# thucz/splatter360

Measured on AMD Instinct MI355X. Metric: Msplats/s fwd+bwd @1M Gaussians, 1024x512 ERP, higher is better.
Workload: dtype f32; 1 GPU; BASELINE configs[2]: 1048576 encoder-like synthetic Gaussians (seed 0, deg-4 SH, from 2 context panoramas 1024x512), 1024x512 ERP = 6 faces 256x256 + stitch, fwdbwd, L2 loss on faces (fused epilogue, scalar reduced in the backward's first launch), lean tile lists; gaussians=1048576, face=256, views_per_gpu=1, parallelism=view-sharded x1, num_rendered=2237238, visible_pairs=1096454, split_lists=auto, split_quadrants=0, wide_rectangles=0, workspace_bytes_forward=1086434304, workspace_bytes_backward=1062934272, max_instances=2862083

## Files before the change

### splatter360_amd/csrc/s360_device.h

```cpp
#pragma once
#include <hip/hip_runtime.h>
#include <stdint.h>

#include "../../include/s360.h"

#define S360_WAVE 64
#define S360_BLOCK 256

#ifndef S360_SUB_W
#define S360_SUB_W 8
#endif

static inline int s360_effective_degree(const S360Params* prm) {
    return (prm->sh_degree > 3 && (prm->flags & S360_FLAG_SH_DEG4_IGNORED)) ? 3 : prm->sh_degree;
}

#ifndef S360_PREC_F4
#define S360_PREC_F4 4
#endif

namespace s360 {

constexpr int PREC_F4 = S360_PREC_F4;
constexpr int SUB_W = S360_SUB_W, SUB_H = 64 / S360_SUB_W;
__device__ __forceinline__ int sub_ox(int w) { return SUB_W == 16 ? 0 : 8 * (w & 1); }
__device__ __forceinline__ int sub_oy(int w) { return SUB_W == 16 ? 4 * w : 8 * (w >> 1); }


struct KParams {
    int P, V, H, W, deg, M;
    int gx, gy, T;
    uint32_t flags, cap;
};

#ifndef S360_SEG_LEN
#define S360_SEG_LEN 512
#endif
#ifndef S360_SEG_HEAD
#define S360_SEG_HEAD 1024
#endif
#ifndef S360_SEG_BWD_BLOCKS
#define S360_SEG_BWD_BLOCKS 256
#endif
#ifndef S360_SEG_MIN_REST
#define S360_SEG_MIN_REST 512
#endif
constexpr uint32_t SEG_LEN = S360_SEG_LEN, SEG_HEAD = S360_SEG_HEAD, SEG_MIN_REST = S360_SEG_MIN_REST, SEG_PER_CHUNK = 4096 / SEG_LEN;
constexpr uint32_t SEG_K0 = SEG_HEAD / SEG_LEN;
static_assert(4096 % SEG_LEN == 0 && SEG_HEAD % SEG_LEN == 0 && SEG_LEN % 64 == 0 && SEG_K0 >= 1, "segments tile the sort's 4 096-key chunks; slot 0 holds the head's state");
__device__ constexpr float SEG_T_FAR = 1.0f / 16.0f;
__host__ __device__ inline size_t seg_slots(size_t cap) { return (size_t)SEG_PER_CHUNK * (cap / 2048 + 1); }
__host__ __device__ inline size_t seg_slots_of(const S360Params* prm) {
    return prm->max_segments ? (size_t)prm->max_segments : seg_slots(prm->max_instances ? prm->max_instances : 1);
}
#define S360_HDR_SPLIT 5
#define S360_HDR_SEGWORK 6
#define S360_HDR_TILES_DONE 24
#define S360_HDR_NLONG 25
#define S360_SEG_CLAIM 0x80000000u
#define S360_HDR_SEGBUFS 32

inline int device_cu_count() {
    static int cached[64] = {};
    int dev = 0;
    if (hipGetDevice(&dev) != hipSuccess || dev < 0 || dev >= 64) return 256;
    if (!cached[dev]) {
        int n = 0;
        if (hipDeviceGetAttribute(&n, hipDeviceAttributeMultiprocessorCount, dev) != hipSuccess || n <= 0) { (void)hipGetLastError(); n = 256; }
        cached[dev] = n;
    }
    return cached[dev];
}

inline int resident_blocks(const void* fn, int block_threads, int slot) {
    static int cached[64][16] = {};
    int dev = 0;
    if (hipGetDevice(&dev) != hipSuccess || dev < 0 || dev >= 64 || slot < 0 || slot >= 16) return 4 * 256;
    if (!cached[dev][slot]) {
        int per_cu = 0;
        if (hipOccupancyMaxActiveBlocksPerMultiprocessor(&per_cu, fn, block_threads, 0) != hipSuccess || per_cu <= 0) { (void)hipGetLastError(); per_cu = 4; }
        cached[dev][slot] = per_cu * device_cu_count();
    }
    return cached[dev][slot];
}

__device__ constexpr float kC0 = 0.28209479177387814f;
__device__ constexpr float kC1 = 0.4886025119029199f;
__device__ constexpr float kC2[5] = {1.0925484305920792f, -1.0925484305920792f, 0.31539156525252005f,
                                     -1.0925484305920792f, 0.5462742152960396f};
__device__ constexpr float kC3[7] = {-0.5900435899266435f, 2.890611442640554f, -0.4570457994644658f,
                                     0.3731763325901154f, -0.4570457994644658f, 1.445305721320277f,
                                     -0.5900435899266435f};
__device__ constexpr float kC4[9] = {2.5033429417967046f, -1.7701307697799304f, 0.9461746957575601f,
                                     -0.6690465435572892f, 0.10578554691520431f, -0.6690465435572892f,
                                     0.47308734787878004f, -1.7701307697799304f, 0.6258357354491761f};

__device__ __forceinline__ void sh_basis(int deg, float x, float y, float z, float* Y) {
    Y[0] = kC0;
    if (deg > 0) {
        Y[1] = -kC1 * y;
        Y[2] = kC1 * z;
        Y[3] = -kC1 * x;
        if (deg > 1) {
            float xx = x * x, yy = y * y, zz = z * z, xy = x * y, yz = y * z, xz = x * z;
            Y[4] = kC2[0] * xy;
            Y[5] = kC2[1] * yz;
            Y[6] = kC2[2] * (2.0f * zz - xx - yy);
            Y[7] = kC2[3] * xz;
            Y[8] = kC2[4] * (xx - yy);
            if (deg > 2) {
                Y[9] = kC3[0] * y * (3.0f * xx - yy);
                Y[10] = kC3[1] * xy * z;
                Y[11] = kC3[2] * y * (4.0f * zz - xx - yy);
                Y[12] = kC3[3] * z * (2.0f * zz - 3.0f * xx - 3.0f * yy);
                Y[13] = kC3[4] * x * (4.0f * zz - xx - yy);
                Y[14] = kC3[5] * z * (xx - yy);
                Y[15] = kC3[6] * x * (xx - 3.0f * yy);
// ... 537 lines not shown
```

### splatter360_amd/csrc/s360_forward.hip

```cpp
#include "s360_device.h"
#include "s360_prof.h"
#include "s360_adapter_math.h"

#include <cstdio>
#include <cstdlib>

namespace s360 {

typedef float f4v __attribute__((ext_vector_type(4)));

template <bool CH_MAJOR, bool JAC>
__global__ __launch_bounds__(S360_BLOCK) void k_sh_eval(KParams kp, const S360View* __restrict__ views,
                                                       const float* __restrict__ means, const float* __restrict__ shs,
                                                       float4* __restrict__ rgbc, float* __restrict__ sh_jac,
                                                       uint32_t* __restrict__ zero_ptr, int zero_words) {
    const int g = blockIdx.x * S360_BLOCK + threadIdx.x;
    if (g < zero_words) zero_ptr[g] = 0u;
    if (g >= kp.P) return;
    const bool fast = kp.M == 25 && kp.deg == 4;
    const float* sh = shs + (size_t)g * kp.M * 3;
    float c[75];
    if (fast) load75(sh, c);
    const S360View& vw = views[0];
    const float sc = vw.scale;
// ... 326 lines not shown
#pragma unroll
        for (int a = 0; a < 3; ++a)
#pragma unroll
            for (int b = a; b < 3; ++b) S[a][b] = S[b][a] = M[a][0] * s2[0] * M[b][0] + M[a][1] * s2[1] * M[b][1] + M[a][2] * s2[2] * M[b][2];
        float* oc = rin.cov6_out + 6 * (size_t)g;
        oc[0] = S[0][0]; oc[1] = S[0][1]; oc[2] = S[0][2]; oc[3] = S[1][1]; oc[4] = S[1][2]; oc[5] = S[2][2];
    }
    if (d == 2 && live && rin.geo7) {
        const float* rw = s_raw + l * RAW_C;
        float* o7 = rin.geo7 + 7 * (size_t)g;
#pragma unroll
        for (int k = 0; k < 7; ++k) o7[k] = rw[k];
    }
    __syncthreads();
    if (JAC) {
        const int gl = tid / 3, ch = tid - 3 * gl;
        if (gl < nb) {
            const float G0 = s_G[(3 * ch) * SHE3_G + gl], G1 = s_G[(3 * ch + 1) * SHE3_G + gl], G2 = s_G[(3 * ch + 2) * SHE3_G + gl];
            const float4 dr = s_dir[gl];
            const float dot = dr.x * G0 + dr.y * G1 + dr.z * G2;
            float* o = sh_jac + 3 * ((size_t)g0 * 3 + tid);
            o[0] = (G0 - dr.x * dot) * dr.w;
            o[1] = (G1 - dr.y * dot) * dr.w;
            o[2] = (G2 - dr.z * dot) * dr.w;
        }
    }
    if (tid < nb) {
        const float a0 = s_rgb[3 * tid], a1 = s_rgb[3 * tid + 1], a2 = s_rgb[3 * tid + 2];
        const uint32_t clampbits = (a0 < 0.f ? 1u : 0u) | (a1 < 0.f ? 2u : 0u) | (a2 < 0.f ? 4u : 0u);
        rgbc[g0 + tid] = make_float4(fmaxf(a0, 0.f), fmaxf(a1, 0.f), fmaxf(a2, 0.f), __uint_as_float(clampbits));
    }
}

template <bool USE_SH, bool CH_MAJOR, bool EAGER = false, bool COOP = false>
__global__ __launch_bounds__(S360_BLOCK) void k_preprocess(
    KParams kp, const S360View* __restrict__ views, const float* __restrict__ means,
    const float* __restrict__ cov6, const float* __restrict__ opac, const float* __restrict__ shs,
    const float* __restrict__ colors, int32_t* __restrict__ radii, uint32_t* __restrict__ tiles_touched,
    float4* __restrict__ recA, float4* __restrict__ recB, float4* __restrict__ recC,
    uint8_t* __restrict__ clamped, float* __restrict__ depths, uint32_t* __restrict__ tile_count, int lds_hist,
    const float4* __restrict__ rgbc, uint8_t* __restrict__ vis_mask, uint2* __restrict__ slot_info) {
    extern __shared__ __attribute__((aligned(16))) float lds_sh[];
    const int tid = threadIdx.x;
    const int g0 = blockIdx.x * S360_BLOCK;
    const int P = kp.P;
    const bool act = g0 + tid < P;
    const int g = act ? g0 + tid : P - 1;
    uint32_t* hist = reinterpret_cast<uint32_t*>(lds_sh);
    const bool lean = (kp.flags & S360_FLAG_LEAN_LISTS) != 0;
    const int nhist = lds_hist == 2 ? kp.T : (image_of_view(kp, kp.V - 1) + 1) * kp.T;
    if (lds_hist)
        for (int i = tid; i < nhist; i += S360_BLOCK) hist[i] = 0u;

    __syncthreads();
    {
    const float mx0 = means[3 * g], my0 = means[3 * g + 1], mz0 = means[3 * g + 2];
    float c60[6];
    load_cov6(cov6, g, (kp.flags & S360_FLAG_COV9) != 0, c60);
    const float op = opac[g];
    constexpr bool ch_major = CH_MAJOR;

    const bool shared_cam = (kp.flags & S360_FLAG_SHARED_CAMPOS) != 0;
    float rgb[3] = {0.f, 0.f, 0.f};
    uint32_t clampbits = 0;
    bool have_rgb = false;
    if (!USE_SH) {
        rgb[0] = colors[3 * g];
        rgb[1] = colors[3 * g + 1];
        rgb[2] = colors[3 * g + 2];
        have_rgb = true;
    }

    uint32_t vis = 0;
    for (int v = 0; v < kp.V; ++v) {
// ... 165 lines not shown
                for (int i = lane; i < n; i += 64) {
                    const int y = i / w;
                    atomicAdd(&tc[(miny + y) * kp.gx + minx + (i - y * w)], 1u);
                }
            }
        }
        if (act && radii) radii[p] = radius;
        if (touched) {
            tiles_touched[p] = touched;
            vis |= 1u << v;
        }
        if (lds_hist == 2) {
            __syncthreads();
            uint32_t* tcg = tile_count + (size_t)image_of_view(kp, v) * kp.T;
            for (int i = tid; i < nhist; i += S360_BLOCK) {
                const uint32_t c = hist[i];
                if (c) {
                    atomicAdd(&tcg[i], c);
                    hist[i] = 0u;
                }
            }
            __syncthreads();
        }
    }
    if (act) vis_mask[g] = (uint8_t)vis;
    }
    if (lds_hist == 1) {
        __syncthreads();
        for (int i = tid; i < nhist; i += S360_BLOCK) {
            const uint32_t c = hist[i];
            if (c) atomicAdd(&tile_count[i], c);
        }
    }
}


template <int NW = S360_BLOCK / 64>
__device__ __forceinline__ uint32_t block_exclusive_scan(uint32_t v, uint32_t* lds, uint32_t& total) {
    const int lane = lane_id(), wave = threadIdx.x >> 6;
    uint32_t inc = v;
#pragma unroll
    for (int o = 1; o < 64; o <<= 1) {
        uint32_t t = (uint32_t)__shfl_up((int)inc, o);
        if (lane >= o) inc += t;
    }
    if (lane == 63) lds[wave] = inc;
    __syncthreads();
    uint32_t base = 0, tot = 0;
#pragma unroll
    for (int w = 0; w < NW; ++w) {
        const uint32_t s = lds[w];
        if (w < wave) base += s;
        tot += s;
    }
    __syncthreads();
    total = tot;
    return base + inc - v;
}

#ifndef S360_SORT_THREADS
#define S360_SORT_THREADS 512
#endif
constexpr int SORT_THREADS = S360_SORT_THREADS;
constexpr uint32_t SORT_SHORT = 2048;
constexpr uint32_t SORT_CHUNK = 8 * SORT_THREADS;
static_assert(SORT_SHORT % SORT_THREADS == 0 && SORT_SHORT <= SORT_CHUNK, "short lists: SORT_SHORT / SORT_THREADS keys per thread");
constexpr uint32_t MAX_PASSES = 4;
__device__ __forceinline__ uint32_t ceil_log2_u32(uint32_t x) { return x <= 1 ? 0u : 32u - (uint32_t)__builtin_clz(x - 1); }
constexpr uint32_t LDSM_CHUNKS = 4;
constexpr int LDSM_E = 32;
__device__ __forceinline__ uint32_t merge_passes_of(uint32_t nch) { return nch <= 1 ? 0u : nch <= LDSM_CHUNKS ? 1u : ceil_log2_u32(nch); }

struct SegBufs {
    const uint32_t* chunk_start;
    uint32_t* seg_flag;
    uint32_t* seg_arrive;
    uint32_t* seg_arrive2;
    uint32_t n_slots;
    float4* part_c;
    float* part_t;
    float* part_e;
    uint32_t* part_l;
    uint32_t* part_n;
    float4* seg_c;
    float* seg_t;
    uint32_t* seg_cnt;
    uint2* seg_info;
    uint32_t* header;
};
static_assert(sizeof(SegBufs) <= (64 - S360_HDR_SEGBUFS) * 4, "SegBufs is parked in the workspace header");

constexpr int TS_BLOCK = 1024;
__global__ __launch_bounds__(TS_BLOCK) void k_tile_scan(const uint32_t* __restrict__ tile_count, uint32_t* __restrict__ tile_start,
                                                         uint32_t* __restrict__ tile_cursor, uint32_t* __restrict__ tile_max_contrib,
                                                         int nt, uint32_t cap, uint32_t* __restrict__ header,
                                                         uint32_t* __restrict__ chunk_start, unsigned long long* __restrict__ header_mirror,
                                                         SegBufs sg_in) {
    __shared__ uint32_t lds[TS_BLOCK / 64];
    __shared__ uint32_t lds_max, lds_nlong;
    if (threadIdx.x == 0) { lds_max = 0; lds_nlong = 0; }
    __syncthreads();
    uint32_t carry = 0, mx = 0, ccarry = 0;
    for (int b = 0; b < nt; b += 2 * TS_BLOCK) {
        const int i0 = b + 2 * (int)threadIdx.x, i1 = i0 + 1;
        uint32_t v0 = 0u, v1 = 0u;
        if (i1 < nt) {
            const uint2 vv = *reinterpret_cast<const uint2*>(tile_count + i0);
            v0 = vv.x; v1 = vv.y;
        } else if (i0 < nt) {
            v0 = tile_count[i0];
        }
        mx = max(mx, max(v0, v1));
        uint32_t tot;
        const uint32_t ex0 = block_exclusive_scan<TS_BLOCK / 64>(v0 + v1, lds, tot), ex1 = ex0 + v0;
        const uint32_t nc0 = min(carry + ex0 + v0, cap) - min(carry + ex0, cap), nc1 = min(carry + ex1 + v1, cap) - min(carry + ex1, cap);
        const uint32_t nch0 = nc0 > SORT_SHORT ? (nc0 + SORT_CHUNK - 1) / SORT_CHUNK : 0u;
        const uint32_t nch1 = nc1 > SORT_SHORT ? (nc1 + SORT_CHUNK - 1) / SORT_CHUNK : 0u;
        if (nch0 || nch1) atomicAdd(&lds_nlong, (nch0 ? 1u : 0u) + (nch1 ? 1u : 0u));
        uint32_t ctot;
        const uint32_t cex0 = block_exclusive_scan<TS_BLOCK / 64>(nch0 + nch1, lds, ctot), cex1 = cex0 + nch0;
        if (i0 < nt) {
            tile_start[i0] = carry + ex0;
            tile_cursor[i0] = 0;
            tile_max_contrib[i0] = 0;
            chunk_start[i0] = ccarry + cex0;
        }
        if (i1 < nt) {
            tile_start[i1] = carry + ex1;
            tile_cursor[i1] = 0;
            tile_max_contrib[i1] = 0;
            chunk_start[i1] = ccarry + cex1;
        }
        carry += tot;
        ccarry += ctot;
    }
    atomicMax(&lds_max, mx);
    __syncthreads();
    if (threadIdx.x == 0) {
        chunk_start[nt] = ccarry;
        tile_start[nt] = carry;
        header[0] = carry;
        header[1] = carry > cap ? 1u : 0u;
        header[2] = lds_max;
        {
            const uint32_t nmax = min(lds_max, cap);
            const uint32_t nch = nmax > SORT_SHORT ? (nmax + SORT_CHUNK - 1) / SORT_CHUNK : 0u;
            header[3] = merge_passes_of(nch);
        }
        header[4] = 0;
        *reinterpret_cast<SegBufs*>(header + S360_HDR_SEGBUFS) = sg_in;
        header[S360_HDR_SPLIT] = 0;
        header[6] = header[7] = 0;
        if (header_mirror) __hip_atomic_store(header_mirror, (unsigned long long)carry | ((unsigned long long)(carry > cap ? 1u : 0u) << 32) |
                                                             ((unsigned long long)ccarry << 33),
                                              __ATOMIC_RELAXED, __HIP_MEMORY_SCOPE_SYSTEM);
        header[S360_HDR_NLONG] = lds_nlong;
        for (int i = 8; i < 25; ++i) header[i] = 0;
    }
}

#ifndef S360_EMIT_PPT
#define S360_EMIT_PPT 4
#endif
constexpr int EMIT_PPT = S360_EMIT_PPT;

template <bool LDS_BIN, bool COOP = false>
__global__ __launch_bounds__(S360_BLOCK) void k_emit(KParams kp, const uint32_t* __restrict__ tiles_touched,
                                                    const uint8_t* __restrict__ vis_mask, const float4* __restrict__ recA, const float4* __restrict__ recC,
                                                    const float* __restrict__ depths, const uint32_t* __restrict__ tile_start,
                                                    uint32_t* __restrict__ tile_cursor, uint64_t* __restrict__ keys,
                                                    uint2* __restrict__ slot_info, uint32_t* __restrict__ slot_pair,
                                                    uint32_t* __restrict__ slot_ticket, uint32_t* __restrict__ header,
                                                    uint32_t* __restrict__ long_pairs) {
    extern __shared__ __attribute__((aligned(16))) uint32_t lds_bin[];
    __shared__ uint32_t s_scan[S360_BLOCK / 64];
    __shared__ uint32_t s_slot0;
    const int v = blockIdx.y;
    const int g0 = blockIdx.x * (S360_BLOCK * EMIT_PPT) + threadIdx.x;
    const size_t tb = (size_t)image_of_view(kp, v) * kp.T;
    uint32_t* cnt = lds_bin;
    uint32_t* base = lds_bin + kp.T;
    const bool lean = (kp.flags & S360_FLAG_LEAN_LISTS) != 0;
    if (LDS_BIN) {
        for (int i = threadIdx.x; i < kp.T; i += S360_BLOCK) cnt[i] = 0u;
        __syncthreads();
    }
    __shared__ uint32_t s_p[S360_BLOCK * EMIT_PPT];
    uint32_t vis = 0;
#pragma unroll
    for (int j = 0; j < EMIT_PPT; ++j) {
// ... 730 lines not shown
                    const bool stop = mine && test_T < 0.0001f;
                    const bool contrib = mine && !stop;
                    if (!T_ONLY) {
                        const float w = contrib ? a_s * T : 0.0f;
                        C01.x += rl(eb.z, eb_) * w;
                        C01.y += rl(eb.w, eb_) * w;
                        C2D.x += rl(ec, eb_) * w;
                        if (WITH_DEPTH) C2D.y += rl(ez, eb_) * w;
                        last = contrib ? rel + (uint32_t)eb_ + 1u : last;
                    }
                    T = contrib ? test_T : T;
                    done = done || stop;
                    if (__ballot(stop) != 0ull) break;
                }
            }
        }
    }
}

template <bool WITH_DEPTH, bool COH>
__device__ __forceinline__ void seg_item(const KParams& kp, const S360View* __restrict__ views, const uint32_t* __restrict__ tile_start,
                                         const uint32_t* __restrict__ list, const float4* __restrict__ recA, float* __restrict__ images,
                                         float* __restrict__ final_T, uint32_t* __restrict__ n_contrib, uint32_t* __restrict__ tile_max_contrib,
                                         uint32_t* __restrict__ strip_last, const float* __restrict__ depths, float* __restrict__ depth_maps,
                                         int depth_mode, const MseEp& ep, float4* __restrict__ surv, uint32_t* __restrict__ surv_count,
                                         const SegBufs& sg, int nt, uint32_t* __restrict__ dbg, const WaveLds& L, int lane, uint2 item, uint32_t wi,
                                         uint32_t nwork);

#ifndef S360_SPLIT_WAVES
#define S360_SPLIT_WAVES 4
#endif
#ifndef S360_P1_GRID
#define S360_P1_GRID 1024
#endif
#ifndef S360_P1_FIRST
#define S360_P1_FIRST 0
#endif
#ifndef S360_P2_GRID
#define S360_P2_GRID 1024
#endif
#ifndef S360_SEGS_SPINS
#define S360_SEGS_SPINS 600
#endif
template <bool WITH_DEPTH, bool SPLIT>
__global__ __launch_bounds__(S360_BLOCK) __attribute__((amdgpu_waves_per_eu(SPLIT ? S360_SPLIT_WAVES : 6, SPLIT ? S360_SPLIT_WAVES : 6))) void k_render(KParams kp, const S360View* __restrict__ views,
                                                      const uint32_t* __restrict__ tile_start, const uint32_t* __restrict__ list,
                                                      const float4* __restrict__ recA, const float4* __restrict__ recB,
                                                      const float4* __restrict__ recC, float* __restrict__ images,
                                                      float* __restrict__ final_T, uint32_t* __restrict__ n_contrib,
                                                      uint32_t* __restrict__ tile_max_contrib, uint32_t* __restrict__ strip_last,
                                                      uint32_t* __restrict__ dbg, const float* __restrict__ depths,
                                                      float* __restrict__ depth_maps, int depth_mode, MseEp ep,
                                                      const uint32_t* __restrict__ tile_order, float4* __restrict__ surv,
                                                      uint32_t* __restrict__ surv_count, uint32_t* __restrict__ hdr_loss,
                                                      const SegBufs* __restrict__ sgp, const uint32_t* __restrict__ chunk_start,
                                                      unsigned long long* __restrict__ cand_mirror, int nt, const uint32_t* __restrict__ list_all,
                                                      const float* __restrict__ depths_all) {
#ifdef S360_DBG_TIMING
    const long long t_begin = wall_clock64();
#endif
    __shared__ __attribute__((aligned(16))) float s_x[S360_BLOCK / 64][68], s_y[S360_BLOCK / 64][68], s_a[S360_BLOCK / 64][68],
        s_b[S360_BLOCK / 64][68], s_c[S360_BLOCK / 64][68], s_o[S360_BLOCK / 64][68];
    __shared__ __attribute__((aligned(16))) float2 s_rg[S360_BLOCK / 64][68], s_bz[S360_BLOCK / 64][68];
    __shared__ __attribute__((aligned(16))) uint32_t s_pos[S360_BLOCK / 64][68];
    if (hdr_loss && blockIdx.x == 0 && threadIdx.x == 0) {
        const uint64_t pp = (uint64_t)(uintptr_t)ep.partials, po = (uint64_t)(uintptr_t)ep.loss_out;
        hdr_loss[0] = (uint32_t)pp; hdr_loss[1] = (uint32_t)(pp >> 32);
        hdr_loss[2] = (uint32_t)po; hdr_loss[3] = (uint32_t)(po >> 32);
        hdr_loss[4] = (uint32_t)(kp.T * 4); hdr_loss[5] = (uint32_t)kp.V;
        hdr_loss[6] = __float_as_uint(0.5f * ep.grad_scale);
        hdr_loss[7] = __float_as_uint(1.0f / (3.0f * (float)kp.H * (float)kp.W));
        for (int i = 0; i <= kp.V; ++i) ep.loss_out[i] = __uint_as_float(0x7FC00000u);
    }
    __shared__ uint32_t s_retired;
    uint32_t tile_slot = blockIdx.x;
    if (SPLIT) {
        const SegBufs& sgr = *sgp;
        const uint32_t n_long = S360_P1_FIRST ? sgr.header[S360_HDR_NLONG] : (uint32_t)nt;
        const uint32_t b = blockIdx.x;
        if (b >= n_long && b < n_long + (uint32_t)S360_P1_GRID) {
            const SegBufs sg = sgr;
            const int pwave = threadIdx.x >> 6, lane = threadIdx.x & 63;
            const WaveLds L{s_x[pwave], s_y[pwave], s_a[pwave], s_b[pwave], s_c[pwave], s_o[pwave], s_rg[pwave], s_bz[pwave], s_pos[pwave]};
            const uint32_t nunits = min((uint32_t)(SEG_PER_CHUNK * chunk_start[nt]), sg.n_slots);
            for (uint32_t u = b - n_long; u < nunits; u += (uint32_t)S360_P1_GRID) {
#ifdef S360_DBG_TIMING
                const long long t_p1 = wall_clock64();
#endif
                const ChunkUnit cu = chunk_unit(tile_start, chunk_start, nt, kp.cap, u / SEG_PER_CHUNK);
                const uint32_t k = cu.k * SEG_PER_CHUNK + (u % SEG_PER_CHUNK);
                if (!cu.valid || k < SEG_K0 || k * SEG_LEN >= cu.n || cu.n < SEG_HEAD + SEG_MIN_REST) continue;
                const int t1 = (int)cu.t, v1 = t1 / kp.T, rem1 = t1 - v1 * kp.T;
                const int ty1 = rem1 / kp.gx, tx1 = rem1 - ty1 * kp.gx;
                const int px1 = tx1 * 16 + sub_ox(pwave) + lane % SUB_W, py1 = ty1 * 16 + sub_oy(pwave) + lane / SUB_W;
                const bool inside1 = px1 < kp.W && py1 < kp.H;
                float T1 = 1.0f;
                f2 c01 = f2{0.f, 0.f}, c2d = f2{0.f, 0.f};
                uint32_t last1 = 0, cnt1 = 0;
                bool done1 = !inside1;
                const uint32_t b0 = cu.s + k * SEG_LEN, b1 = min(b0 + SEG_LEN, cu.s + cu.n);
                composite_segment<WITH_DEPTH, true>(list, recA, depths, cu.s, b0, b1, (float)px1, (float)py1, (float)(tx1 * 16 + sub_ox(pwave)),
                                                    (float)(ty1 * 16 + sub_oy(pwave)), lane, L, 0.f, 0.f, 0.f, depth_mode, T1, c01, c2d, last1, done1,
                                                    nullptr, cnt1);
                st_devf(sg.part_t + ((size_t)u * 4 + pwave) * 64 + lane, (done1 && inside1) ? 0.0f : T1);
                asm volatile("s_waitcnt vmcnt(0)" ::: "memory");
                if (lane == 0) __hip_atomic_fetch_add(&sg.seg_arrive[4 * t1 + pwave], 1u, __ATOMIC_RELAXED, __HIP_MEMORY_SCOPE_AGENT);
#ifdef S360_DBG_TIMING
                if (lane == 0) {
                    const size_t di = 4 * ((size_t)4 * nt + (size_t)4 * sg.n_slots + (size_t)u * 4 + pwave);
                    dbg[di] = (uint32_t)t_begin; dbg[di + 1] = (uint32_t)t_p1; dbg[di + 2] = (uint32_t)(wall_clock64() - t_p1);
                    dbg[di + 3] = ((uint32_t)t1 << 8) | k;
// ... 709 lines not shown
    if (sph && (kp.V & 1)) return S360_E_BADARG;
    const int nt = (sph ? kp.V / 2 : kp.V) * kp.T;
    const size_t np = (size_t)kp.V * kp.P;

    uint32_t* header = (uint32_t*)(ws + L.header);
    uint32_t* tiles_touched = (uint32_t*)(ws + L.tiles_touched);
    uint8_t* vis_mask = (uint8_t*)(ws + L.vis_mask);
    uint2* slot_info = (uint2*)(ws + L.slot_base);
    uint32_t* slot_ticket = (uint32_t*)(ws + L.slot_ticket);
    float4* recA = (float4*)(ws + L.rec_a);
    float4* recB = (float4*)(ws + L.rec_b);
    float4* recC = (float4*)(ws + L.rec_c);
    uint8_t* clamped = (uint8_t*)(ws + L.clamped);
    float* depths = (float*)(ws + L.depths);
    uint32_t* tile_count = (uint32_t*)(ws + L.tile_count);
    uint32_t* tile_start = (uint32_t*)(ws + L.tile_start);
    uint32_t* tile_cursor = (uint32_t*)(ws + L.tile_cursor);
    uint64_t* keys = (uint64_t*)(ws + L.keys);
    uint64_t* keys_alt = (uint64_t*)(ws + L.keys_alt);
    uint32_t* chunk_start = (uint32_t*)(ws + L.chunk_start);
    uint32_t* tile_order = (uint32_t*)(ws + L.tile_order);
    uint32_t* list = (uint32_t*)(ws + L.list);
    float* final_T = (float*)(ws + L.final_T);
    uint32_t* n_contrib = (uint32_t*)(ws + L.n_contrib);
    uint32_t* tile_max_contrib = (uint32_t*)(ws + L.tile_max_contrib);
    uint32_t* strip_last = (uint32_t*)(ws + L.strip_last);

    const bool eager_sh = kp.P > 0 && shs && (kp.flags & S360_FLAG_SHARED_CAMPOS) && (!(kp.flags & S360_FLAG_FORWARD_ONLY) || kp.V >= 2 || rawin);
    const size_t zero_words_sz = (L.tile_start - L.tile_count) / 4;
    const bool fold_clear = eager_sh && zero_words_sz <= (size_t)kp.P;
    uint32_t* zero_ptr = fold_clear ? tile_count : (uint32_t*)nullptr;
    const int zero_words = fold_clear ? (int)zero_words_sz : 0;
    if (!fold_clear && hipMemsetAsync(tile_count, 0, L.tile_start - L.tile_count, st) != hipSuccess) return S360_E_LAUNCH;
    if (kp.P > 0) {
        {
        const int nblk = (kp.P + S360_BLOCK - 1) / S360_BLOCK;
        const int lds_hist = (size_t)nt * 4 <= 48 * 1024 ? 1 : ((size_t)kp.T * 4 <= 48 * 1024 ? 2 : 0);
        const size_t hist_bytes = lds_hist == 2 ? (size_t)kp.T * 4 : (size_t)nt * 4;
        const bool eager = eager_sh;
        float4* rgbc = (float4*)(ws + L.rgbc);
        if (eager) {
            ProfScope ps(PS_SH_EVAL, st);
            float* sh_jac = (float*)(ws + L.sh_jac);
            const bool jac = !(kp.flags & S360_FLAG_FORWARD_ONLY);
            const bool chm = (kp.flags & S360_FLAG_SH_CHANNEL_MAJOR) != 0;
#define S360_SHE(A, B) hipLaunchKernelGGL((k_sh_eval<A, B>), dim3(nblk), dim3(S360_BLOCK), 0, st, kp, views, means3D, shs, rgbc, sh_jac, zero_ptr, zero_words)
            if (rawin) {
                RawIn rin = *rawin;
                rin.geo7 = jac ? (float*)(ws + L.geo7) : nullptr;
                const dim3 rgrid((rin.Gv + SHE3_G - 1) / SHE3_G, (unsigned)(kp.P / rin.Gv));
                const bool rot = rin.sh_rot != nullptr;
#define S360_RAWE(J, R, M) hipLaunchKernelGGL((k_raw_eval<J, R, M>), rgrid, dim3(SHE3_G * 3), 0, st, kp, views, rin, rgbc, sh_jac, zero_ptr, zero_words)
                static const bool raw_mfma = [] { const char* e = getenv("S360_RAW_MFMA"); return e && e[0] == '1'; }();
                if (rot && raw_mfma) { if (jac) S360_RAWE(true, true, true); else S360_RAWE(false, true, true); }
                else if (jac) { if (rot) S360_RAWE(true, true, false); else S360_RAWE(true, false, false); }
                else { if (rot) S360_RAWE(false, true, false); else S360_RAWE(false, false, false); }
#undef S360_RAWE
            } else if (chm && kp.M == 25 && kp.deg == 4) {
                const int nb3 = (kp.P + SHE3_G - 1) / SHE3_G;
                if (jac) hipLaunchKernelGGL(k_sh_eval3_jac, dim3(nb3), dim3(SHE3_G * 3), 0, st, kp, views, means3D, shs, rgbc, sh_jac, zero_ptr, zero_words);
                else hipLaunchKernelGGL(k_sh_eval3, dim3(nb3), dim3(SHE3_G * 3), 0, st, kp, views, means3D, shs, rgbc, zero_ptr, zero_words);
            } else if (chm && jac) S360_SHE(true, true); else if (chm) S360_SHE(true, false); else if (jac) S360_SHE(false, true); else S360_SHE(false, false);
#undef S360_SHE
        }
        ProfScope ps(PS_PREPROCESS, st);
        if (shs) {
            const size_t lds = lds_hist ? hist_bytes : 0;
            if (eager && (kp.flags & S360_FLAG_COOP_WALK))
                hipLaunchKernelGGL((k_preprocess<true, true, true, true>), dim3(nblk), dim3(S360_BLOCK), lds, st, kp, views, means3D, cov6,
                                   opacities, shs, colors_precomp, radii, tiles_touched, recA, recB, recC, clamped, depths,
                                   tile_count, lds_hist, rgbc, vis_mask, slot_info);
            else if (eager)
                hipLaunchKernelGGL((k_preprocess<true, true, true>), dim3(nblk), dim3(S360_BLOCK), lds, st, kp, views, means3D, cov6,
                                   opacities, shs, colors_precomp, radii, tiles_touched, recA, recB, recC, clamped, depths,
                                   tile_count, lds_hist, rgbc, vis_mask, slot_info);
            else if (kp.flags & S360_FLAG_SH_CHANNEL_MAJOR)
                hipLaunchKernelGGL((k_preprocess<true, true>), dim3(nblk), dim3(S360_BLOCK), lds, st, kp, views, means3D, cov6,
                                   opacities, shs, colors_precomp, radii, tiles_touched, recA, recB, recC, clamped, depths,
                                   tile_count, lds_hist, rgbc, vis_mask, slot_info);
            else
                hipLaunchKernelGGL((k_preprocess<true, false>), dim3(nblk), dim3(S360_BLOCK), lds, st, kp, views, means3D, cov6,
                                   opacities, shs, colors_precomp, radii, tiles_touched, recA, recB, recC, clamped, depths,
                                   tile_count, lds_hist, rgbc, vis_mask, slot_info);
        } else {
            hipLaunchKernelGGL((k_preprocess<false, false>), dim3(nblk), dim3(S360_BLOCK), lds_hist ? hist_bytes : 0, st, kp, views,
                               means3D, cov6, opacities, shs, colors_precomp, radii, tiles_touched, recA, recB, recC, clamped,
                               depths, tile_count, lds_hist, rgbc, vis_mask, slot_info);
        }
        }
        S360_CHECK_LAUNCH();
    }
    {
        ProfScope ps(PS_TILE_SCAN, st);
        const bool split0 = kp.P > 0 && (kp.flags & S360_FLAG_SPLIT_LISTS);
        SegBufs sg0{split0 ? chunk_start : (const uint32_t*)nullptr, (uint32_t*)(ws + L.seg_flag), (uint32_t*)(ws + L.seg_arrive),
                    (uint32_t*)(ws + L.seg_arrive2), (uint32_t)seg_slots_of(prm),
                    (float4*)(ws + L.part_c), (float*)(ws + L.part_t), (float*)(ws + L.part_e), (uint32_t*)(ws + L.part_l), (uint32_t*)(ws + L.part_n),
                    (float4*)(ws + L.seg_c), (float*)(ws + L.seg_t), (uint32_t*)(ws + L.seg_cnt), (uint2*)(ws + L.seg_info), header};
        hipLaunchKernelGGL(k_tile_scan, dim3(1), dim3(TS_BLOCK), 0, st, tile_count, tile_start, tile_cursor, tile_max_contrib, nt, kp.cap, header,
                           chunk_start, (unsigned long long*)prm->header_mirror, sg0);
    }
    S360_CHECK_LAUNCH();
    if (kp.P > 0) {
        const dim3 egrid((kp.P + S360_BLOCK * EMIT_PPT - 1) / (S360_BLOCK * EMIT_PPT), kp.V);
        uint32_t* slot_pair = (kp.flags & S360_FLAG_FORWARD_ONLY) ? nullptr : (uint32_t*)(ws + L.slot_pair);
        {
        ProfScope ps(PS_EMIT, st);
        if ((size_t)kp.T * 8 <= 64 * 1024 && (kp.flags & S360_FLAG_COOP_WALK))
            hipLaunchKernelGGL((k_emit<true, true>), egrid, dim3(S360_BLOCK), (size_t)kp.T * 8, st, kp, tiles_touched, vis_mask, recA, recC,
                               depths, tile_start, tile_cursor, keys, slot_info, slot_pair, slot_ticket, header, (uint32_t*)(ws + L.long_pairs));
        else if ((size_t)kp.T * 8 <= 64 * 1024)
            hipLaunchKernelGGL(k_emit<true>, egrid, dim3(S360_BLOCK), (size_t)kp.T * 8, st, kp, tiles_touched, vis_mask, recA, recC,
                               depths, tile_start, tile_cursor, keys, slot_info, slot_pair, slot_ticket, header, (uint32_t*)(ws + L.long_pairs));
        else
            hipLaunchKernelGGL(k_emit<false>, egrid, dim3(S360_BLOCK), 0, st, kp, tiles_touched, vis_mask, recA, recC, depths, tile_start,
                               tile_cursor, keys, slot_info, slot_pair, slot_ticket, header, (uint32_t*)(ws + L.long_pairs));
        }
        S360_CHECK_LAUNCH();
        ProfScope ps(PS_SORT, st);
        {
            const size_t cap_keys = kp.cap < (uint32_t)kp.P ? kp.cap : (size_t)kp.P;
            uint32_t passes = 0;
            while (passes < MAX_PASSES && ((size_t)SORT_CHUNK << passes) < cap_keys) ++passes;
            const uint32_t global_lo = SORT_CHUNK << passes;
            const unsigned cgrid = (unsigned)min((size_t)1024, (size_t)kp.cap / SORT_CHUNK + (size_t)kp.cap / SORT_SHORT + 2);
            const size_t lds512 = (size_t)(SORT_CHUNK + SORT_CHUNK / 8) * 8;
            hipLaunchKernelGGL(k_sort_stage1, dim3(cgrid + nt + 1), dim3(SORT_THREADS), lds512, st, tile_start, chunk_start, nt, keys, keys_alt, list,
                               kp.cap, passes, cgrid, tile_count, tile_order, header,
                               prm->header_mirror ? (unsigned long long*)prm->header_mirror + 2 : (unsigned long long*)nullptr);
            if (passes > 0) {
                const unsigned mgrid = cgrid < (unsigned)S360_MERGE_GRID ? cgrid : (unsigned)S360_MERGE_GRID;
                {
                    static bool attr_done[64] = {};
// ... 108 lines not shown
```

Baseline: 1355 Msplats/s.

## Fold tile-count scan into the last preprocess workgroup to drop a launch

The single-block tile scan kernel is removed from the normal path. Instead, each preprocess workgroup increments a done counter after its histogram flush, and the last one to finish runs the scan body itself, reading its arguments from the kernarg segment. This removes one kernel launch and the dependency gap before the scan. In exchange the scan runs on a 256-thread block instead of 1024 threads, and the optional long-tile count header field and the P1_FIRST path are dropped.

Result: slower. 1338 Msplats/s (-1.3%).

```diff
diff --git a/splatter360_amd/csrc/s360_device.h b/splatter360_amd/csrc/s360_device.h
--- a/splatter360_amd/csrc/s360_device.h
+++ b/splatter360_amd/csrc/s360_device.h
@@ -56,33 +56,8 @@
 #define S360_HDR_SPLIT 5
 #define S360_HDR_SEGWORK 6
 #define S360_HDR_TILES_DONE 24
-#define S360_HDR_NLONG 25
 #define S360_SEG_CLAIM 0x80000000u
 #define S360_HDR_SEGBUFS 32
-
-inline int device_cu_count() {
-    static int cached[64] = {};
-    int dev = 0;
-    if (hipGetDevice(&dev) != hipSuccess || dev < 0 || dev >= 64) return 256;
-    if (!cached[dev]) {
-        int n = 0;
-        if (hipDeviceGetAttribute(&n, hipDeviceAttributeMultiprocessorCount, dev) != hipSuccess || n <= 0) { (void)hipGetLastError(); n = 256; }
-        cached[dev] = n;
-    }
-    return cached[dev];
-}
-
-inline int resident_blocks(const void* fn, int block_threads, int slot) {
-    static int cached[64][16] = {};
-    int dev = 0;
-    if (hipGetDevice(&dev) != hipSuccess || dev < 0 || dev >= 64 || slot < 0 || slot >= 16) return 4 * 256;
-    if (!cached[dev][slot]) {
-        int per_cu = 0;
-        if (hipOccupancyMaxActiveBlocksPerMultiprocessor(&per_cu, fn, block_threads, 0) != hipSuccess || per_cu <= 0) { (void)hipGetLastError(); per_cu = 4; }
-        cached[dev][slot] = per_cu * device_cu_count();
-    }
-    return cached[dev][slot];
-}
 
 __device__ constexpr float kC0 = 0.28209479177387814f;
 __device__ constexpr float kC1 = 0.4886025119029199f;
diff --git a/splatter360_amd/csrc/s360_forward.hip b/splatter360_amd/csrc/s360_forward.hip
--- a/splatter360_amd/csrc/s360_forward.hip
+++ b/splatter360_amd/csrc/s360_forward.hip
@@ -382,6 +382,195 @@
     }
 }
 
+
+template <int NW = S360_BLOCK / 64>
+__device__ __forceinline__ uint32_t block_exclusive_scan(uint32_t v, uint32_t* lds, uint32_t& total) {
+    const int lane = lane_id(), wave = threadIdx.x >> 6;
+    uint32_t inc = v;
+#pragma unroll
+    for (int o = 1; o < 64; o <<= 1) {
+        uint32_t t = (uint32_t)__shfl_up((int)inc, o);
+        if (lane >= o) inc += t;
+    }
+    if (lane == 63) lds[wave] = inc;
+    __syncthreads();
+    uint32_t base = 0, tot = 0;
+#pragma unroll
+    for (int w = 0; w < NW; ++w) {
+        const uint32_t s = lds[w];
+        if (w < wave) base += s;
+        tot += s;
+    }
+    __syncthreads();
+    total = tot;
+    return base + inc - v;
+}
+
+#ifndef S360_SORT_THREADS
+#define S360_SORT_THREADS 512
+#endif
+constexpr int SORT_THREADS = S360_SORT_THREADS;
+constexpr uint32_t SORT_SHORT = 2048;
+constexpr uint32_t SORT_CHUNK = 8 * SORT_THREADS;
+static_assert(SORT_SHORT % SORT_THREADS == 0 && SORT_SHORT <= SORT_CHUNK, "short lists: SORT_SHORT / SORT_THREADS keys per thread");
+constexpr uint32_t MAX_PASSES = 4;
+__device__ __forceinline__ uint32_t ceil_log2_u32(uint32_t x) { return x <= 1 ? 0u : 32u - (uint32_t)__builtin_clz(x - 1); }
+constexpr uint32_t LDSM_CHUNKS = 4;
+constexpr int LDSM_E = 32;
+__device__ __forceinline__ uint32_t merge_passes_of(uint32_t nch) { return nch <= 1 ? 0u : nch <= LDSM_CHUNKS ? 1u : ceil_log2_u32(nch); }
+
+struct SegBufs {
+    const uint32_t* chunk_start;
+    uint32_t* seg_flag;
+    uint32_t* seg_arrive;
+    uint32_t* seg_arrive2;
+    uint32_t n_slots;
+    float4* part_c;
+    float* part_t;
+    float* part_e;
+    uint32_t* part_l;
+    uint32_t* part_n;
+    float4* seg_c;
+    float* seg_t;
+    uint32_t* seg_cnt;
+    uint2* seg_info;
+    uint32_t* header;
+};
+static_assert(sizeof(SegBufs) <= (64 - S360_HDR_SEGBUFS) * 4, "SegBufs is parked in the workspace header");
+
+__device__ __forceinline__ uint32_t sort_chunks_of(uint32_t nc0) {
+    const uint32_t nch0 = nc0 > SORT_SHORT ? (nc0 + SORT_CHUNK - 1) / SORT_CHUNK : 0u;
+    return nch0;
+}
+
+struct ScanArgs {
+    const uint32_t* tile_count;
+    uint32_t* tile_start;
+    uint32_t* tile_cursor;
+    uint32_t* tile_max_contrib;
+    uint32_t* chunk_start;
+    uint32_t* header;
+    unsigned long long* header_mirror;
+    uint32_t* done;
+    int nt;
+    uint32_t cap;
+    SegBufs sg;
+};
+
+__device__ __forceinline__ uint32_t ld_count(const uint32_t* p) { return __hip_atomic_load(p, __ATOMIC_RELAXED, __HIP_MEMORY_SCOPE_AGENT); }
+
+template <int THREADS>
+__device__ __forceinline__ void tile_scan_body(const ScanArgs& sa, uint32_t* lds) {
+    constexpr int PER = 8;
+    uint32_t* lds_max = lds + THREADS / 64;
+    if (threadIdx.x == 0) *lds_max = 0;
+    __syncthreads();
+    const int nt = sa.nt;
+    const uint32_t cap = sa.cap;
+    uint32_t carry = 0, mx = 0, ccarry = 0;
+    for (int b = 0; b < nt; b += PER * THREADS) {
+        const int i0 = b + PER * (int)threadIdx.x;
+        uint32_t v[PER], sum = 0;
+#pragma unroll
+        for (int k = 0; k < PER; ++k) v[k] = i0 + k < nt ? ld_count(sa.tile_count + i0 + k) : 0u;
+#pragma unroll
+        for (int k = 0; k < PER; ++k) {
+            mx = max(mx, v[k]);
+            sum += v[k];
+        }
+        uint32_t tot;
+        const uint32_t ex = carry + block_exclusive_scan<THREADS / 64>(sum, lds, tot);
+        uint32_t nch[PER], csum = 0, off = ex;
+#pragma unroll
+        for (int k = 0; k < PER; ++k) {
+            const uint32_t nc = min(off + v[k], cap) - min(off, cap);
+            nch[k] = sort_chunks_of(nc);
+            csum += nch[k];
+            off += v[k];
+        }
+        uint32_t ctot;
+        uint32_t coff = ccarry + block_exclusive_scan<THREADS / 64>(csum, lds, ctot);
+        off = ex;
+#pragma unroll
+        for (int k = 0; k < PER; ++k) {
+            if (i0 + k < nt) {
+                sa.tile_start[i0 + k] = off;
+                sa.tile_cursor[i0 + k] = 0;
+                sa.tile_max_contrib[i0 + k] = 0;
+                sa.chunk_start[i0 + k] = coff;
+            }
+            off += v[k];
+            coff += nch[k];
+        }
+        carry += tot;
+        ccarry += ctot;
+    }
+    atomicMax(lds_max, mx);
+    __syncthreads();
+    if (threadIdx.x == 0) {
+        uint32_t* header = sa.header;
+        sa.chunk_start[nt] = ccarry;
+        sa.tile_start[nt] = carry;
+        header[0] = carry;
+        header[1] = carry > cap ? 1u : 0u;
+        header[2] = *lds_max;
+        {
+            const uint32_t nmax = min(*lds_max, cap);
+            header[3] = merge_passes_of(sort_chunks_of(nmax));
+        }
+        header[4] = 0;
+        {
+            SegBufs* d = reinterpret_cast<SegBufs*>(header + S360_HDR_SEGBUFS);
+            d->chunk_start = sa.sg.chunk_start; d->seg_flag = sa.sg.seg_flag; d->seg_arrive = sa.sg.seg_arrive; d->seg_arrive2 = sa.sg.seg_arrive2;
+            d->n_slots = sa.sg.n_slots; d->part_c = sa.sg.part_c; d->part_t = sa.sg.part_t; d->part_e = sa.sg.part_e; d->part_l = sa.sg.part_l;
+            d->part_n = sa.sg.part_n; d->seg_c = sa.sg.seg_c; d->seg_t = sa.sg.seg_t; d->seg_cnt = sa.sg.seg_cnt; d->seg_info = sa.sg.seg_info;
+            d->header = sa.sg.header;
+        }
+        header[S360_HDR_SPLIT] = 0;
+        header[6] = header[7] = 0;
+        if (sa.header_mirror) __hip_atomic_store(sa.header_mirror, (unsigned long long)carry | ((unsigned long long)(carry > cap ? 1u : 0u) << 32) |
+                                                                   ((unsigned long long)ccarry << 33),
+                                                 __ATOMIC_RELAXED, __HIP_MEMORY_SCOPE_SYSTEM);
+        for (int i = 8; i < 25; ++i) header[i] = 0;
+    }
+}
+
+constexpr int TS_BLOCK = 256;
+__global__ __launch_bounds__(TS_BLOCK) void k_tile_scan(ScanArgs sa) {
+    __shared__ uint32_t lds[TS_BLOCK / 64 + 1];
+    tile_scan_body<TS_BLOCK>(sa, lds);
+}
+
+__device__ __forceinline__ bool last_workgroup(uint32_t* done, uint32_t* s_flag) {
+    __builtin_amdgcn_s_waitcnt(0x0F70);
+    __syncthreads();
+    if (threadIdx.x == 0) {
+        const bool last = __hip_atomic_fetch_add(done, 1u, __ATOMIC_RELAXED, __HIP_MEMORY_SCOPE_AGENT) == gridDim.x - 1;
+        if (last) __hip_atomic_store(done, 0u, __ATOMIC_RELAXED, __HIP_MEMORY_SCOPE_AGENT);
+        *s_flag = last ? 1u : 0u;
+    }
+    __syncthreads();
+    return *s_flag != 0u;
+}
+
+struct PreprocessKernargs {
+    KParams kp;
+    const S360View* views;
+    const float *means, *cov6, *opac, *shs, *colors;
+    int32_t* radii;
+    uint32_t* tiles_touched;
+    float4 *recA, *recB, *recC;
+    uint8_t* clamped;
+    float* depths;
+    uint32_t* tile_count;
+    int lds_hist;
+    const float4* rgbc;
+    uint8_t* vis_mask;
+    uint2* slot_info;
+    ScanArgs sa;
+};
+__host__ __device__ inline size_t scan_done_word(int nt) { return ((size_t)nt * 4 + 255) / 256 * 64 + 1; }
+__device__ __forceinline__ size_t scan_done_word(const KParams& kp) { return scan_done_word(kp.V * kp.T); }
 template <bool USE_SH, bool CH_MAJOR, bool EAGER = false, bool COOP = false>
 __global__ __launch_bounds__(S360_BLOCK) void k_preprocess(
     KParams kp, const S360View* __restrict__ views, const float* __restrict__ means,
@@ -389,7 +578,8 @@
     const float* __restrict__ colors, int32_t* __restrict__ radii, uint32_t* __restrict__ tiles_touched,
     float4* __restrict__ recA, float4* __restrict__ recB, float4* __restrict__ recC,
     uint8_t* __restrict__ clamped, float* __restrict__ depths, uint32_t* __restrict__ tile_count, int lds_hist,
-    const float4* __restrict__ rgbc, uint8_t* __restrict__ vis_mask, uint2* __restrict__ slot_info) {
+    const float4* __restrict__ rgbc, uint8_t* __restrict__ vis_mask, uint2* __restrict__ slot_info, ScanArgs sa_) {
+    (void)sa_;
     extern __shared__ __attribute__((aligned(16))) float lds_sh[];
     const int tid = threadIdx.x;
     const int g0 = blockIdx.x * S360_BLOCK;
@@ -621,130 +811,12 @@
             if (c) atomicAdd(&tile_count[i], c);
         }
     }
-}
-
-
-template <int NW = S360_BLOCK / 64>
-__device__ __forceinline__ uint32_t block_exclusive_scan(uint32_t v, uint32_t* lds, uint32_t& total) {
-    const int lane = lane_id(), wave = threadIdx.x >> 6;
-    uint32_t inc = v;
-#pragma unroll
-    for (int o = 1; o < 64; o <<= 1) {
-        uint32_t t = (uint32_t)__shfl_up((int)inc, o);
-        if (lane >= o) inc += t;
-    }
-    if (lane == 63) lds[wave] = inc;
-    __syncthreads();
-    uint32_t base = 0, tot = 0;
-#pragma unroll
-    for (int w = 0; w < NW; ++w) {
-        const uint32_t s = lds[w];
-        if (w < wave) base += s;
-        tot += s;
-    }
-    __syncthreads();
-    total = tot;
-    return base + inc - v;
-}
-
-#ifndef S360_SORT_THREADS
-#define S360_SORT_THREADS 512
-#endif
-constexpr int SORT_THREADS = S360_SORT_THREADS;
-constexpr uint32_t SORT_SHORT = 2048;
-constexpr uint32_t SORT_CHUNK = 8 * SORT_THREADS;
-static_assert(SORT_SHORT % SORT_THREADS == 0 && SORT_SHORT <= SORT_CHUNK, "short lists: SORT_SHORT / SORT_THREADS keys per thread");
-constexpr uint32_t MAX_PASSES = 4;
-__device__ __forceinline__ uint32_t ceil_log2_u32(uint32_t x) { return x <= 1 ? 0u : 32u - (uint32_t)__builtin_clz(x - 1); }
-constexpr uint32_t LDSM_CHUNKS = 4;
-constexpr int LDSM_E = 32;
-__device__ __forceinline__ uint32_t merge_passes_of(uint32_t nch) { return nch <= 1 ? 0u : nch <= LDSM_CHUNKS ? 1u : ceil_log2_u32(nch); }
-
-struct SegBufs {
-    const uint32_t* chunk_start;
-    uint32_t* seg_flag;
-    uint32_t* seg_arrive;
-    uint32_t* seg_arrive2;
-    uint32_t n_slots;
-    float4* part_c;
-    float* part_t;
-    float* part_e;
-    uint32_t* part_l;
-    uint32_t* part_n;
-    float4* seg_c;
-    float* seg_t;
-    uint32_t* seg_cnt;
-    uint2* seg_info;
-    uint32_t* header;
-};
-static_assert(sizeof(SegBufs) <= (64 - S360_HDR_SEGBUFS) * 4, "SegBufs is parked in the workspace header");
-
-constexpr int TS_BLOCK = 1024;
-__global__ __launch_bounds__(TS_BLOCK) void k_tile_scan(const uint32_t* __restrict__ tile_count, uint32_t* __restrict__ tile_start,
-                                                         uint32_t* __restrict__ tile_cursor, uint32_t* __restrict__ tile_max_contrib,
-                                                         int nt, uint32_t cap, uint32_t* __restrict__ header,
-                                                         uint32_t* __restrict__ chunk_start, unsigned long long* __restrict__ header_mirror,
-                                                         SegBufs sg_in) {
-    __shared__ uint32_t lds[TS_BLOCK / 64];
-    __shared__ uint32_t lds_max, lds_nlong;
-    if (threadIdx.x == 0) { lds_max = 0; lds_nlong = 0; }
-    __syncthreads();
-    uint32_t carry = 0, mx = 0, ccarry = 0;
-    for (int b = 0; b < nt; b += 2 * TS_BLOCK) {
-        const int i0 = b + 2 * (int)threadIdx.x, i1 = i0 + 1;
-        uint32_t v0 = 0u, v1 = 0u;
-        if (i1 < nt) {
-            const uint2 vv = *reinterpret_cast<const uint2*>(tile_count + i0);
-            v0 = vv.x; v1 = vv.y;
-        } else if (i0 < nt) {
-            v0 = tile_count[i0];
-        }
-        mx = max(mx, max(v0, v1));
-        uint32_t tot;
-        const uint32_t ex0 = block_exclusive_scan<TS_BLOCK / 64>(v0 + v1, lds, tot), ex1 = ex0 + v0;
-        const uint32_t nc0 = min(carry + ex0 + v0, cap) - min(carry + ex0, cap), nc1 = min(carry + ex1 + v1, cap) - min(carry + ex1, cap);
-        const uint32_t nch0 = nc0 > SORT_SHORT ? (nc0 + SORT_CHUNK - 1) / SORT_CHUNK : 0u;
-        const uint32_t nch1 = nc1 > SORT_SHORT ? (nc1 + SORT_CHUNK - 1) / SORT_CHUNK : 0u;
-        if (nch0 || nch1) atomicAdd(&lds_nlong, (nch0 ? 1u : 0u) + (nch1 ? 1u : 0u));
-        uint32_t ctot;
-        const uint32_t cex0 = block_exclusive_scan<TS_BLOCK / 64>(nch0 + nch1, lds, ctot), cex1 = cex0 + nch0;
-        if (i0 < nt) {
-            tile_start[i0] = carry + ex0;
-            tile_cursor[i0] = 0;
-            tile_max_contrib[i0] = 0;
-            chunk_start[i0] = ccarry + cex0;
-        }
-        if (i1 < nt) {
-            tile_start[i1] = carry + ex1;
-            tile_cursor[i1] = 0;
-            tile_max_contrib[i1] = 0;
-            chunk_start[i1] = ccarry + cex1;
-        }
-        carry += tot;
-        ccarry += ctot;
-    }
-    atomicMax(&lds_max, mx);
-    __syncthreads();
-    if (threadIdx.x == 0) {
-        chunk_start[nt] = ccarry;
-        tile_start[nt] = carry;
-        header[0] = carry;
-        header[1] = carry > cap ? 1u : 0u;
-        header[2] = lds_max;
-        {
-            const uint32_t nmax = min(lds_max, cap);
-            const uint32_t nch = nmax > SORT_SHORT ? (nmax + SORT_CHUNK - 1) / SORT_CHUNK : 0u;
-            header[3] = merge_passes_of(nch);
-        }
-        header[4] = 0;
-        *reinterpret_cast<SegBufs*>(header + S360_HDR_SEGBUFS) = sg_in;
-        header[S360_HDR_SPLIT] = 0;
-        header[6] = header[7] = 0;
-        if (header_mirror) __hip_atomic_store(header_mirror, (unsigned long long)carry | ((unsigned long long)(carry > cap ? 1u : 0u) << 32) |
-                                                             ((unsigned long long)ccarry << 33),
-                                              __ATOMIC_RELAXED, __HIP_MEMORY_SCOPE_SYSTEM);
-        header[S360_HDR_NLONG] = lds_nlong;
-        for (int i = 8; i < 25; ++i) header[i] = 0;
+    __shared__ uint32_t s_scan[S360_BLOCK / 64 + 2];
+    const ScanArgs& sa = *reinterpret_cast<const ScanArgs*>(reinterpret_cast<const char*>((const void*)__builtin_amdgcn_kernarg_segment_ptr()) +
+                                                            offsetof(PreprocessKernargs, sa));
+    if (last_workgroup(tile_count + scan_done_word(kp), &s_scan[S360_BLOCK / 64 + 1])) {
+        if (sa.tile_count != tile_count) __builtin_trap();
+        tile_scan_body<S360_BLOCK>(sa, s_scan);
     }
 }
 
@@ -1541,9 +1613,6 @@
 #endif
 #ifndef S360_P1_GRID
 #define S360_P1_GRID 1024
-#endif
-#ifndef S360_P1_FIRST
-#define S360_P1_FIRST 0
 #endif
 #ifndef S360_P2_GRID
 #define S360_P2_GRID 1024
@@ -1585,7 +1654,7 @@
     uint32_t tile_slot = blockIdx.x;
     if (SPLIT) {
         const SegBufs& sgr = *sgp;
-        const uint32_t n_long = S360_P1_FIRST ? sgr.header[S360_HDR_NLONG] : (uint32_t)nt;
+        const uint32_t n_long = (uint32_t)nt;
         const uint32_t b = blockIdx.x;
         if (b >= n_long && b < n_long + (uint32_t)S360_P1_GRID) {
             const SegBufs sg = sgr;
@@ -2361,6 +2430,14 @@
     uint32_t* zero_ptr = fold_clear ? tile_count : (uint32_t*)nullptr;
     const int zero_words = fold_clear ? (int)zero_words_sz : 0;
     if (!fold_clear && hipMemsetAsync(tile_count, 0, L.tile_start - L.tile_count, st) != hipSuccess) return S360_E_LAUNCH;
+    if (tile_count + scan_done_word(kp.V * kp.T) != slot_ticket + 1) return S360_E_BADARG;
+    const bool split0 = kp.P > 0 && (kp.flags & S360_FLAG_SPLIT_LISTS);
+    const ScanArgs sa{tile_count, tile_start, tile_cursor, tile_max_contrib, chunk_start, header, (unsigned long long*)prm->header_mirror,
+                      slot_ticket + 1, nt, kp.cap,
+                      SegBufs{split0 ? chunk_start : (const uint32_t*)nullptr, (uint32_t*)(ws + L.seg_flag), (uint32_t*)(ws + L.seg_arrive),
+                              (uint32_t*)(ws + L.seg_arrive2), (uint32_t)seg_slots_of(prm),
+                              (float4*)(ws + L.part_c), (float*)(ws + L.part_t), (float*)(ws + L.part_e), (uint32_t*)(ws + L.part_l), (uint32_t*)(ws + L.part_n),
+                              (float4*)(ws + L.seg_c), (float*)(ws + L.seg_t), (uint32_t*)(ws + L.seg_cnt), (uint2*)(ws + L.seg_info), header}};
     if (kp.P > 0) {
         {
         const int nblk = (kp.P + S360_BLOCK - 1) / S360_BLOCK;
@@ -2398,36 +2475,30 @@
             if (eager && (kp.flags & S360_FLAG_COOP_WALK))
                 hipLaunchKernelGGL((k_preprocess<true, true, true, true>), dim3(nblk), dim3(S360_BLOCK), lds, st, kp, views, means3D, cov6,
                                    opacities, shs, colors_precomp, radii, tiles_touched, recA, recB, recC, clamped, depths,
-                                   tile_count, lds_hist, rgbc, vis_mask, slot_info);
+                                   tile_count, lds_hist, rgbc, vis_mask, slot_info, sa);
             else if (eager)
                 hipLaunchKernelGGL((k_preprocess<true, true, true>), dim3(nblk), dim3(S360_BLOCK), lds, st, kp, views, means3D, cov6,
                                    opacities, shs, colors_precomp, radii, tiles_touched, recA, recB, recC, clamped, depths,
-                                   tile_count, lds_hist, rgbc, vis_mask, slot_info);
+                                   tile_count, lds_hist, rgbc, vis_mask, slot_info, sa);
             else if (kp.flags & S360_FLAG_SH_CHANNEL_MAJOR)
                 hipLaunchKernelGGL((k_preprocess<true, true>), dim3(nblk), dim3(S360_BLOCK), lds, st, kp, views, means3D, cov6,
                                    opacities, shs, colors_precomp, radii, tiles_touched, recA, recB, recC, clamped, depths,
-                                   tile_count, lds_hist, rgbc, vis_mask, slot_info);
+                                   tile_count, lds_hist, rgbc, vis_mask, slot_info, sa);
             else
                 hipLaunchKernelGGL((k_preprocess<true, false>), dim3(nblk), dim3(S360_BLOCK), lds, st, kp, views, means3D, cov6,
                                    opacities, shs, colors_precomp, radii, tiles_touched, recA, recB, recC, clamped, depths,
-                                   tile_count, lds_hist, rgbc, vis_mask, slot_info);
+                                   tile_count, lds_hist, rgbc, vis_mask, slot_info, sa);
         } else {
             hipLaunchKernelGGL((k_preprocess<false, false>), dim3(nblk), dim3(S360_BLOCK), lds_hist ? hist_bytes : 0, st, kp, views,
                                means3D, cov6, opacities, shs, colors_precomp, radii, tiles_touched, recA, recB, recC, clamped,
-                               depths, tile_count, lds_hist, rgbc, vis_mask, slot_info);
+                               depths, tile_count, lds_hist, rgbc, vis_mask, slot_info, sa);
         }
         }
         S360_CHECK_LAUNCH();
     }
-    {
+    if (kp.P <= 0) {
         ProfScope ps(PS_TILE_SCAN, st);
-        const bool split0 = kp.P > 0 && (kp.flags & S360_FLAG_SPLIT_LISTS);
-        SegBufs sg0{split0 ? chunk_start : (const uint32_t*)nullptr, (uint32_t*)(ws + L.seg_flag), (uint32_t*)(ws + L.seg_arrive),
-                    (uint32_t*)(ws + L.seg_arrive2), (uint32_t)seg_slots_of(prm),
-                    (float4*)(ws + L.part_c), (float*)(ws + L.part_t), (float*)(ws + L.part_e), (uint32_t*)(ws + L.part_l), (uint32_t*)(ws + L.part_n),
-                    (float4*)(ws + L.seg_c), (float*)(ws + L.seg_t), (uint32_t*)(ws + L.seg_cnt), (uint2*)(ws + L.seg_info), header};
-        hipLaunchKernelGGL(k_tile_scan, dim3(1), dim3(TS_BLOCK), 0, st, tile_count, tile_start, tile_cursor, tile_max_contrib, nt, kp.cap, header,
-                           chunk_start, (unsigned long long*)prm->header_mirror, sg0);
+        hipLaunchKernelGGL(k_tile_scan, dim3(1), dim3(TS_BLOCK), 0, st, sa);
     }
     S360_CHECK_LAUNCH();
     if (kp.P > 0) {
```
